# claudiok/clsim

Measured on AMD Instinct MI355X. Metric: propagated photons/sec (whole node), higher is better.
Workload: dtype f32

## Files before the change

clsim_amd/csrc/c_api.cpp:

```cpp
#include <cstring>
#include <map>
#include <memory>
#include <mutex>

#include "converter.h"
#include "lightsource.h"
#include "feeder.h"
#include "tabulator.h"
#include "step_store.h"
#include "flasher.h"
#include "mcpe.h"
#include "mcpe_merge.h"
#include "mcpe_union.h"
#include "pmt_hits.h"
#include "cable_shadow.h"
#include "event_stats.h"
#include "frame_photons.h"
#include "frame_photon_union.h"
#include "pmt_series.h"
#include "photon_hits.h"
#include "pmt_photon_hits.h"

using namespace clsimhip;

// ... 586 lines not shown
    long n = 0;
    const int rc = guarded_const(c, [&] { need(c, "converter"); need(name, "name"); n = c->impl.get_table(name, out, cap); });
    return rc == CLSIMHIP_OK ? n : rc;
}
static void copy_launched(const clsimhip::KLaunched &l, int out[6])
{
    out[0] = l.family; out[1] = l.lengths; out[2] = l.tilt; out[3] = l.aniso; out[4] = l.flasher; out[5] = l.fast;
}
int clsimhip_get_last_launch(const clsimhip_converter *c, int out[6])
{
    return guarded_const(c, [&] { need(c, "converter"); need(out, "out"); copy_launched(c->impl.last_launch(), out); });
}
int clsimhip_get_rng_state(clsimhip_converter *c, uint64_t *x_out, size_t count)
{
    return guarded(c, [&] { need(c, "converter"); c->impl.get_rng_state(x_out, count); });
}
int clsimhip_debug_counters(clsimhip_converter *c, uint32_t out[4])
{
    return guarded(c, [&] { need(c, "converter"); c->impl.debug_counters(out); });
}
int clsimhip_eval_device_function(clsimhip_converter *c, int what, int layer, int fast, const float *in4, size_t n, float *out4)
{
    return guarded(c, [&] { need(c, "converter"); c->impl.eval_device_function(what, layer, fast != 0, in4, n, out4); });
}
int clsimhip_eval_device_random(clsimhip_converter *c, int what, int generator, int fast, uint64_t *x, const uint32_t *a, size_t n_streams, size_t draws,
                                float *out)
{
    return guarded(c, [&] { need(c, "converter"); c->impl.eval_device_random(what, generator, fast != 0, x, a, n_streams, draws, out); });
}
int clsimhip_eval_math(int device_ordinal, int what, const float *x, const float *y, size_t n, float *out)
{
    return guarded(nullptr, [&] {
        need(x, "x"); need(out, "out");
        int count = 0;
        if (hipGetDeviceCount(&count) != hipSuccess || count <= 0) throw Error(CLSIMHIP_ERR_DEVICE, "no HIP device available");
        DeviceGuard on_device(device_ordinal);
        DeviceBuffer<float> bx(n + 4, "hipMalloc"), by, bout(n + 4, "hipMalloc");
        float *dx = bx.get(), *dy = nullptr, *dout = bout.get();
        hip_check(hipMemcpy(dx, x, n * 4, hipMemcpyHostToDevice), "hipMemcpy");
        if (y) {
            by.alloc(n + 4, "hipMalloc");
            dy = by.get();
            hip_check(hipMemcpy(dy, y, n * 4, hipMemcpyHostToDevice), "hipMemcpy");
        }
        hip_check(launch_eval_math(what, dx, dy, static_cast<uint32_t>(n), dout, nullptr), "eval_math launch");
        hip_check(hipDeviceSynchronize(), "eval_math");
        hip_check(hipMemcpy(out, dout, n * 4, hipMemcpyDeviceToHost), "hipMemcpy");
    });
}
int clsimhip_check_math_exhaustive(int device_ordinal, int what, int exp_lo, int exp_hi, uint32_t *result, size_t result_cap)
{
    return guarded(nullptr, [&] {
        need(result, "result");
        if (!((what >= 11 && what <= 13) || (what >= 16 && what <= 19)) || exp_lo < -126 || exp_hi > 127 || exp_lo > exp_hi || result_cap < 1 || result_cap > 4096)
            throw Error(CLSIMHIP_ERR_CONFIG, "clsimhip_check_math_exhaustive: what in 11..13 or 16..19, -126 <= exp_lo <= exp_hi <= 127, 1 <= result_cap <= 4096");
        int count = 0;
        if (hipGetDeviceCount(&count) != hipSuccess || count <= 0) throw Error(CLSIMHIP_ERR_DEVICE, "no HIP device available");
        DeviceGuard on_device(device_ordinal);
        DeviceBuffer<uint32_t> buf(result_cap, "hipMalloc");
        hip_check(hipMemset(buf.get(), 0, result_cap * 4), "hipMemset");
        hip_check(launch_check_math(what, exp_lo, exp_hi, buf.get(), static_cast<uint32_t>(result_cap), nullptr), "check_math launch");
        hip_check(hipDeviceSynchronize(), "check_math");
        hip_check(hipMemcpy(result, buf.get(), result_cap * 4, hipMemcpyDeviceToHost), "hipMemcpy");
    });
}


namespace {
void plan_steps(const clsimhip_step_request *requests, size_t n, size_t granularity, std::vector<uint64_t> &first, uint64_t &real, uint64_t &padded)
{
    need(requests, "requests");
    if (granularity == 0) throw Error(CLSIMHIP_ERR_ARGUMENT, "granularity must not be 0");
    first.assign(n + 1, 0);
    for (size_t i = 0; i < n; ++i) {
        const clsimhip_step_request &q = requests[i];
        if (q.kind > CLSIMHIP_STEPS_MUON) throw Error(CLSIMHIP_ERR_ARGUMENT, "unknown step request kind");
        if (q.photons_per_step == 0 && q.num_steps > 0) throw Error(CLSIMHIP_ERR_ARGUMENT, "photonsPerStep may not be <= 0!");
        if (q.kind == CLSIMHIP_STEPS_CASCADE && !(q.pa > 0.f)) throw Error(CLSIMHIP_ERR_ARGUMENT, "cascade shape parameter must be positive");
        first[i + 1] = first[i] + q.num_steps + (q.num_photons_in_last_step > 0 ? 1 : 0);
    }
    real = first[n];
    padded = ((real + granularity - 1) / granularity) * granularity;
}
}

extern "C" {
int clsimhip_count_generated_steps(const clsimhip_step_request *requests, size_t n, size_t granularity, size_t *steps_out, size_t *padded_out)
{
    return guarded(nullptr, [&] {
        std::vector<uint64_t> first; uint64_t real = 0, padded = 0;
        plan_steps(requests, n, granularity, first, real, padded);
        if (steps_out) *steps_out = static_cast<size_t>(real);
        if (padded_out) *padded_out = static_cast<size_t>(padded);
    });
}
int clsimhip_generate_steps_device(int device, const clsimhip_step_request *requests, size_t n, uint64_t seed, size_t granularity,
                                   void *d_steps, size_t capacity, void *hip_stream, size_t *padded_out)
{
    return guarded(nullptr, [&] {
        need(d_steps, "d_steps");
        std::vector<uint64_t> first; uint64_t real = 0, padded = 0;
        plan_steps(requests, n, granularity, first, real, padded);
        if (padded > capacity) throw Error(CLSIMHIP_ERR_ARGUMENT, "the requests produce more steps than the buffer holds");
        if (padded_out) *padded_out = static_cast<size_t>(padded);
        if (padded == 0) return;
        int count = 0;
        if (hipGetDeviceCount(&count) != hipSuccess || count <= 0) throw Error(CLSIMHIP_ERR_DEVICE, "no HIP device available (the step producer has no CPU fallback)");
        DeviceGuard on_device(device);
// ... 767 lines not shown
```

clsim_amd/csrc/detmath.hip.h:

```cpp
#pragma once
#ifndef __HIPCC_RTC__
#include <hip/hip_runtime.h>
#include <stdint.h>
#endif

#include "math_tables.h"

#define DM __device__ __forceinline__

namespace dm {

DM float fma_(float a, float b, float c) { return __builtin_fmaf(a, b, c); }
DM float sqrt_(float a) { return __builtin_sqrtf(a); }
DM float rsqrt_(float a) { return 1.0f / __builtin_sqrtf(a); }
DM float rint_(float a) { return __builtin_rintf(a); }

DM uint32_t f2u(float f) { return __builtin_bit_cast(uint32_t, f); }
DM float u2f(uint32_t u) { return __builtin_bit_cast(float, u); }

DM float rcp_(float x)
{
    const float r0 = __builtin_amdgcn_rcpf(x);
    const float e0 = fma_(-x, r0, 1.0f);
    return fma_(e0, r0, r0);
}
DM float rcp_of_rcp_(float b, float x)
{
    const float e = fma_(-b, x, 1.0f);
    return fma_(e, x, x);
}
DM bool div_near_ok_(float a) { return __builtin_fabsf(a) >= 9.094947017729282e-13f; }
DM float div_near_with_(float a, float b, float y)
{
    const float q0 = a * y;
    const float r0 = fma_(-b, q0, a);
    const float q1 = fma_(r0, y, q0);
    const float r1 = fma_(-b, q1, a);
    return fma_(r1, y, q1);
}
DM float div_near_(float a, float b) { return div_near_with_(a, b, rcp_(b)); }
DM float sqrt_near_(float x)
{
    const float s = __builtin_amdgcn_sqrtf(x);
    const uint32_t dn = __builtin_elementwise_sub_sat(f2u(s), 1u);
    const float s_dn = u2f(dn), s_up = u2f(f2u(s) + 1u);
    const float r_dn = fma_(-s_dn, s, x);
    const float r_up = fma_(-s_up, s, x);
    uint32_t m_dn, m_up;
    asm("v_med3_i32 %0, %1, 0, 1" : "=v"(m_dn) : "v"(r_dn));
    asm("v_med3_i32 %0, %1, 0, 1" : "=v"(m_up) : "v"(r_up));
    return u2f(dn + m_dn + m_up);
}
DM float rsqrt_near_(float x) { return rcp_(sqrt_near_(x)); }
DM bool rsqrt_unit_ok_(float x) { return (f2u(x) - (0x3f800000u - 1023u)) <= 2046u; }
DM float rsqrt_unit_(float x)
{
    const int d = (int)(f2u(x) - 0x3f800000u);
    const uint32_t above = 0x3f800000u - ((uint32_t)d & ~1u);
    const uint32_t below = 0x3f800000u + ((uint32_t)(3 - d) >> 2);
    return u2f((d < 0) ? below : above);
}

constexpr uint32_t kMathLogWords = 4u * MT_LOG_ROWS, kMathScWords = 2u * MT_SC_ROWS, kMathTableWords = (kMathLogWords + kMathScWords + 3u) & ~3u;
static __device__ const float kLogTable[kMathLogWords] = MT_LOG_TABLE;
static __device__ const float kScTable[kMathScWords] = MT_SC_TABLE;
static const float kLogTableHost[kMathLogWords] = MT_LOG_TABLE;
static const float kScTableHost[kMathScWords] = MT_SC_TABLE;

constexpr float LN2_HI = 0.693359375f;
constexpr float LN2_LO = -2.12194440e-4f;
constexpr float LOG2E = 1.44269504088896341f;

DM float log_poly(float r)
{
    float p = 7.0376836292e-2f;
    p = fma_(p, r, -1.1514610310e-1f);
    p = fma_(p, r, 1.1676998740e-1f);
    p = fma_(p, r, -1.2420140846e-1f);
    p = fma_(p, r, 1.4249322787e-1f);
    p = fma_(p, r, -1.6668057665e-1f);
    p = fma_(p, r, 2.0000714765e-1f);
    p = fma_(p, r, -2.4999993993e-1f);
    p = fma_(p, r, 3.3333331174e-1f);
    return p;
}

DM float frexp_sqrt2(float x, int &e)
{
    const uint32_t ix = f2u(x);
    const int32_t d = (int32_t)(ix - 0x3f3504f3u);
    e = d >> 23;
    return u2f(ix - ((uint32_t)e << 23));
}

struct LdsTable { uint32_t address; };
template <class Row> DM Row table_row_(const float *table, uint32_t byte_offset)
{
    return *reinterpret_cast<const Row *>(reinterpret_cast<const char *>(table) + byte_offset);
}
template <class Row> DM Row table_row_(LdsTable table, uint32_t byte_offset)
{
    typedef const Row __attribute__((address_space(3))) *lds_row_ptr;
    return *reinterpret_cast<lds_row_ptr>(static_cast<uintptr_t>(table.address + byte_offset));
}

template <class Table>
DM float log_with_(float x, Table table)
{
    typedef float row_t __attribute__((ext_vector_type(4)));
    const uint32_t ix = f2u(x);
    const float m = u2f((ix & 0x007fffffu) | 0x3f800000u);
    const float fe = (float)__builtin_amdgcn_frexp_expf(x);
    const row_t row = table_row_<row_t>(table, (ix >> 14) & 0x1f0u);
// ... 206 lines not shown
```

clsim_amd/csrc/prop_aux_kernels.hip:

```cpp
#include <hip/hip_runtime.h>

#include "prop_device.hip.h"
#include "prop_launch.h"

namespace clsimhip {

__global__ void __launch_bounds__(256) scan_steps_kernel(const DevStep *steps, uint32_t n, uint32_t *meta, WorkRecord *work,
                                                         const uint64_t *rng_x, const uint32_t *rng_a, uint32_t num_generators)
{
    uint32_t m = 0;
    for (uint32_t i = blockIdx.x * 256 + threadIdx.x; i < n; i += gridDim.x * 256) {
        WorkRecord r;
        r.step = steps[i];
        r.x = rng_x[i];
        r.a = rng_a[i];
        r.done = 0u;
        {
            const float f[8] = {r.step.x, r.step.y, r.step.z, r.step.t, r.step.theta, r.step.phi, r.step.length, r.step.beta};
            bool finite = true;
#pragma unroll
            for (int k = 0; k < 8; ++k) finite = finite && (__builtin_fabsf(f[k]) <= 3.0e38f);
            const bool no_spectrum = (num_generators > 1u) && ((r.step.source_type_and_pad & 0xffu) >= num_generators);
            if ((!finite || no_spectrum) && r.step.num_photons != 0u) { r.step.num_photons = 0u; atomicAdd(meta + 2, 1u); }
        }
// ... 134 lines not shown
                        const uint32_t k2 = atomicAdd(result, 1u);
                        if (k2 + 2u < result_cap && (k2 & 1u) == 0u) { result[k2 + 1u] = dm::f2u(a); result[k2 + 2u] = dm::f2u(b); }
                    }
                }
            }
        }
        return;
    }
    for (int e = exp_lo; e <= exp_hi; ++e) {
        const uint32_t bits = ((uint32_t)(e + 127) << 23) | m;
        for (int sign = 0; sign < ((what == 11 || what == 17) ? 2 : 1); ++sign) {
            const float x = dm::u2f(bits | ((uint32_t)sign << 31));
            float want, got;
            if (what == 18) {
                if (e != exp_lo || sign != 0 || m > 2046u) continue;
                const float xx = dm::u2f(0x3f800000u - 1023u + m);
                want = 1.0f / __builtin_sqrtf(xx); got = dm::rsqrt_unit_(xx);
                if (!dm::rsqrt_unit_ok_(xx) || dm::rsqrt_unit_ok_(dm::u2f(0x3f800000u + 1024u)) || dm::rsqrt_unit_ok_(dm::u2f(0x3f800000u - 1024u))) got = 0.0f;
                if (dm::f2u(want) != dm::f2u(got)) { const uint32_t k = atomicAdd(result, 1u); if (k + 1u < result_cap) result[k + 1u] = dm::f2u(xx); }
                continue;
            }
            if (what == 17) { const float b = 1.0f / x; want = 1.0f / b; got = dm::rcp_of_rcp_(dm::rcp_(x), x); }
            else if (what == 11) { want = 1.0f / x; got = dm::rcp_(x); }
            else if (what == 12) { want = __builtin_sqrtf(x); got = dm::sqrt_near_(x); }
            else { want = 1.0f / __builtin_sqrtf(x); got = dm::rsqrt_near_(x); }
            if (dm::f2u(want) != dm::f2u(got)) {
                const uint32_t k = atomicAdd(result, 1u);
                if (k + 1u < result_cap) result[k + 1u] = dm::f2u(x);
            }
        }
    }
}

hipError_t launch_scan_steps(const KParams &P, hipStream_t stream)
{
    const uint32_t sgrid = (P.n_steps + 255u) / 256u;
    hipLaunchKernelGGL(scan_steps_kernel, dim3(sgrid < 1024u ? sgrid : 1024u), dim3(256), 0, stream, P.steps, P.n_steps, P.queue,
                       P.work, P.rng_x, P.rng_a, (uint32_t)P.num_gen);
    return hipGetLastError();
}

hipError_t launch_assemble_hits(const KParams &P, bool flasher, hipStream_t stream)
{
    const size_t image_bytes = (size_t)P.table_words * 4;
    const void *kernel = flasher ? reinterpret_cast<const void *>(&assemble_hits_kernel<true>) : reinterpret_cast<const void *>(&assemble_hits_kernel<false>);
    if (const hipError_t e = allow_dynamic_lds(kernel, image_bytes)) return e;
    if (flasher) hipLaunchKernelGGL((assemble_hits_kernel<true>), dim3(512), dim3(256), image_bytes, stream, P);
    else hipLaunchKernelGGL((assemble_hits_kernel<false>), dim3(512), dim3(256), image_bytes, stream, P);
    return hipGetLastError();
}

hipError_t launch_check_math(int what, int exp_lo, int exp_hi, uint32_t *result, uint32_t result_cap, hipStream_t stream)
{
    hipLaunchKernelGGL(check_math_kernel, dim3((1u << 23) / 256), dim3(256), 0, stream, what, exp_lo, exp_hi, result, result_cap);
    return hipGetLastError();
}

hipError_t launch_eval_math(int what, const float *xs, const float *ys, uint32_t n, float *out, hipStream_t stream)
{
    if (n == 0) return hipSuccess;
    hipLaunchKernelGGL(eval_math_kernel, dim3((n + 255) / 256), dim3(256), 0, stream, what, xs, ys, n, out);
    return hipGetLastError();
}

}
```

clsim_amd/csrc/prop_device.hip.h:

```cpp
#pragma once
#ifndef __HIPCC_RTC__
#include <hip/hip_runtime.h>
#endif

#include "detmath.hip.h"
#include "../../include/clsimhip.h"
#include "kparams.h"
#include "instrument.hip.h"

namespace clsimhip {

#ifndef CLSIMHIP_BLOCK
#define CLSIMHIP_BLOCK 256
#define CLSIMHIP_MIN_WAVES 7
#endif
constexpr int kBlock = CLSIMHIP_BLOCK;
constexpr int kMinWavesPerSimd = CLSIMHIP_MIN_WAVES;
constexpr int kWavesPerBlock = kBlock / 64;
constexpr int kStageRecords = 8;
constexpr int kStubWords = 16;
#ifndef CLSIMHIP_PRIO_SHIFT
#define CLSIMHIP_PRIO_SHIFT 1
#endif
constexpr int kPrioShift = CLSIMHIP_PRIO_SHIFT;
constexpr int kTabSlots = 512;
#ifndef CLSIMHIP_TAB_POOL
#define CLSIMHIP_TAB_POOL 448
#endif
constexpr int kTabPool = CLSIMHIP_TAB_POOL;
constexpr int kTabSegWords = 12;
constexpr int kTabWaveWords = 2 * kTabPool + 2 * 64 * kTabSegWords;
static_assert(kTabWaveWords >= 2 * kTabSlots + 64 && kTabWaveWords % 4 == 0, "table maker: a wave's LDS region");
constexpr float kEpsilon = 0.00001f;
constexpr float kSpeedOfLight = 0.299792458f;
constexpr float kPi = 3.14159265359f;
constexpr uint32_t kNoStep = 0xffffffffu;
constexpr int kTiltScalarBins = 6;

typedef const __attribute__((address_space(4))) KParams *KP;

DM KP fresh_params(KP p)
{
    asm volatile("" : "+s"(p));
    return p;
}

extern __shared__ __attribute__((aligned(16))) uint32_t lds_words[];

DM uint64_t ballot(bool p) { return __builtin_amdgcn_ballot_w64(p); }

struct Rec4 { float a, b, c, d; };

enum CensusRegion { kCensusCrossing = 0, kCensusFilter = 1, kCensusLiu = 2, kCensusHG = 3, kCensusSearchFull = 4, kCensusSearchNamed = 5,
                    kCensusCreation = 6, kCensusService = 7, kCensusScatter = 8, kCensusWalk = 9, kCensusAim = 10, kCensusRegions = 16 };

DM float lds_log(float x) { return dm::log_with_(x, dm::LdsTable{0u}); }
DM void lds_sincos_2pi(float x, float &s, float &c) { dm::sincos_2pi_with_(x, s, c, dm::LdsTable{4u * dm::kMathLogWords}); }

DM float ldsf(uint32_t i) { return __builtin_bit_cast(float, lds_words[i]); }
DM uint32_t ldsu(uint32_t i) { return lds_words[i]; }
DM Rec4 lds_rec4(uint32_t i) { return *reinterpret_cast<const Rec4 *>(&lds_words[i]); }
#ifdef KPARAMS_BAKED
DM Rec4 lds_rec4_wide(uint32_t i)
{
    typedef float f32x4 __attribute__((ext_vector_type(4)));
    typedef const f32x4 __attribute__((address_space(3))) *lds_vec_ptr;
    const f32x4 v = *reinterpret_cast<lds_vec_ptr>(static_cast<uintptr_t>(4u * i));
    return Rec4{v.x, v.y, v.z, v.w};
}
DM float ldsf_at_byte(uint32_t byte)
{
    typedef const float __attribute__((address_space(3))) *lds_float_ptr;
    return *reinterpret_cast<lds_float_ptr>(static_cast<uintptr_t>(byte));
}
#endif
DM uint32_t lds_u16(uint32_t off, uint32_t i)
{
    const uint32_t w = lds_words[off + (i >> 1)];
    return (i & 1) ? (w >> 16) : (w & 0xffffu);
}

DM float rng_co(uint64_t &x, uint32_t a)
{
    x = (x & 0xffffffffull) * (uint64_t)a + (x >> 32);
    const uint32_t lo = (uint32_t)x;
    float t;
    asm volatile("s_setreg_imm32_b32 hwreg(HW_REG_MODE, 0, 2), 3\n\t"
                 "v_cvt_f32_u32_e32 %0, %1\n\t"
                 "s_setreg_imm32_b32 hwreg(HW_REG_MODE, 0, 2), 0"
                 : "=v"(t) : "v"(lo));
    return t * 2.3283064365386963e-10f;
}
DM float rng_oc(uint64_t &x, uint32_t a) { return 1.0f - rng_co(x, a); }

DM float sqr(float a) { return a * a; }
DM float div_by(float a, float b, float r, bool ok)
{
    if (ok) {
        const float q = a * r;
        return dm::fma_(dm::fma_(-b, q, a), r, q);
    }
    return a / b;
}
DM float rcp_sel(float x, bool fast) { return fast ? dm::rcp_(x) : 1.0f / x; }
constexpr uint32_t kFastLengths = 32u, kFastMatrices = 64u, kFastAniso = 128u;
template <bool FAST>
DM float div_by_t(float a, float b, float r, bool ok)
{
    if (FAST) { const float q = a * r; return dm::fma_(dm::fma_(-b, q, a), r, q); }
    return div_by(a, b, r, ok);
}
template <bool FAST>
DM float rcp_t(float x, bool fast) { return FAST ? dm::rcp_(x) : rcp_sel(x, fast); }
DM float clampf(float v, float lo, float hi) { v = (v > lo) ? v : lo; return (v < hi) ? v : hi; }
DM int clampi(int v, int lo, int hi) { v = (v > lo) ? v : lo; return (v < hi) ? v : hi; }
DM float clampf_ordered(float v, float lo, float hi) { return __builtin_amdgcn_fmed3f(v, lo, hi); }
DM int clamp_index(int v, int hi)
{
#ifdef KPARAMS_BAKED
    if (__builtin_constant_p(hi)) return clampi(v, 0, hi);
#endif
// ... 167 lines not shown
}
template <bool FAST = false>
DM float scattering_cos(KP P, uint64_t &x, uint32_t a)
{
    const ScatterK K = scatter_constants(P);
    const float rr = rng_co(x, a);
    if (!FAST) {
        const int kind = P->scatter_kind;
        if (kind == 0) return hg_cos(K, rr);
        if (kind == 1) return liu_cos(K, rr);
    }
    const uint32_t ok = FAST ? 0xffu : K.div_ok;
    CENSUS_REGION(P, kCensusScatter);
    if (rr < K.mix_frac) {
        CENSUS_REGION(P, kCensusLiu);
        return liu_cos<FAST>(K, div_by_t<FAST>(rr, K.mix_frac, K.rcp_mix_frac, (ok & 4u) != 0));
    }
    CENSUS_REGION(P, kCensusHG);
    return hg_cos<FAST>(K, div_by_t<FAST>(1.0f - rr, K.mix_frac_rest, K.rcp_mix_frac_rest, (ok & 8u) != 0));
}

template <bool FAST = false>
DM float abs_len_corr(KP P, const Vec3 &d)
{
    const float n0 = (P->an_azx * d.x) + (P->an_azy * d.y);
    const float n1 = (P->an_mazy * d.x) + (P->an_azx * d.y);
    const float s0 = n0 * n0, s1 = n1 * n1, s2 = d.z * d.z;
    const float nB = (s0 * P->an_rl[0] + s1 * P->an_rl[1]) + s2 * P->an_rl[2];
    const float An = (s0 * P->an_l[0] + s1 * P->an_l[1]) + s2 * P->an_l[2];
    const float x = (P->an_B2 - nB) * An;
    return (FAST || (P->div_ok & kFastAniso) != 0u) ? 2.0f * dm::rcp_(x) : 2.0f / x;
}
template <typename M>
DM void apply_matrix(M m, int renorm, Vec3 &d, bool fast)
{
    const float x = (m[0] * d.x) + (m[1] * d.y) + (m[2] * d.z);
    const float y = (m[3] * d.x) + (m[4] * d.y) + (m[5] * d.z);
    const float z = (m[6] * d.x) + (m[7] * d.y) + (m[8] * d.z);
    d.x = x; d.y = y; d.z = z;
    if (renorm) {
        const float n2 = d.x * d.x + d.y * d.y + d.z * d.z;
        const float norm = fast ? dm::rsqrt_near_(n2) : dm::rsqrt_(n2);
        d.x = d.x * norm; d.y = d.y * norm; d.z = d.z * norm;
    }
}

template <bool FAST = false>
DM float tilt_z_shift(KP P, float px, float py, float pz)
{
    const float z_rescaled = div_by_t<FAST>(pz - P->tilt_first_z, P->tilt_dz, P->rcp_tilt_dz, (P->div_ok & 1u) != 0);
    const int nz = P->tilt_nz, nd = P->tilt_nd;
    const uint32_t off_dist = P->off_tilt_dist;
#ifdef KPARAMS_BAKED
    const int k = clamp_index((int)z_rescaled, nz - 2);
#else
    const int k = clamp_index((int)__builtin_floorf(z_rescaled), nz - 2);
#endif
    const float fraction_z_above = z_rescaled - (float)k;
    const float fraction_z_below = 1.0f - fraction_z_above;
    const float nr = P->tilt_lnx * px + P->tilt_lny * py;
    int j = 1;
    if (FAST || nd <= kTiltScalarBins + 2) {
#ifdef KPARAMS_BAKED
#pragma unroll
        for (int t = 0; t < kTiltScalarBins; ++t)
            if (t < nd - 2) j += (nr >= P->tilt_inner_dist[t]) ? 1 : 0;
#else
#pragma unroll
        for (int t = 0; t < kTiltScalarBins; ++t) j += (nr >= P->tilt_inner_dist[t]) ? 1 : 0;
#endif
    } else {
        for (int t = 1; t < nd - 1; ++t) j += (nr >= ldsf(off_dist + t)) ? 1 : 0;
    }
#ifdef KPARAMS_BAKED
    const Rec4 bin = (KParams::off_tilt_bins % 4u == 0u) ? lds_rec4_wide(P->off_tilt_bins + 4u * (uint32_t)j) : lds_rec4(P->off_tilt_bins + 4u * (uint32_t)j);
#else
    const Rec4 bin = lds_rec4(P->off_tilt_bins + 4u * (uint32_t)j);
#endif
    const float thisDist = bin.a;
    const float q = (thisDist - nr) * bin.c;
    float frac_at_lower = dm::fma_(dm::fma_(-bin.b, q, thisDist - nr), bin.c, q);
    if (!FAST && __builtin_bit_cast(uint32_t, bin.d) == 0u) frac_at_lower = (thisDist - nr) / bin.b;
    const float frac_at_upper = 1.0f - frac_at_lower;
#ifdef KPARAMS_BAKED
    if (FAST) {
        const uint32_t at = (__builtin_bit_cast(uint32_t, bin.d) >> 1) + 4u * (uint32_t)k;
        const uint32_t up = 4u * (uint32_t)nz;
        const float val_at_lower = (ldsf_at_byte(at + 4u) * fraction_z_above + ldsf_at_byte(at) * fraction_z_below);
        const float val_at_upper = (ldsf_at_byte(at + up + 4u) * fraction_z_above + ldsf_at_byte(at + up) * fraction_z_below);
        return (val_at_upper * frac_at_upper + val_at_lower * frac_at_lower);
    }
#endif
    const uint32_t lo = P->off_tilt_zcorr + (uint32_t)((j - 1) * nz + k);
    const uint32_t hi = lo + (uint32_t)nz;
    const float val_at_lower = (ldsf(lo + 1) * fraction_z_above + ldsf(lo) * fraction_z_below);
    const float val_at_upper = (ldsf(hi + 1) * fraction_z_above + ldsf(hi) * fraction_z_below);
    return (val_at_upper * frac_at_upper + val_at_lower * frac_at_lower);
}

DM float generate_wavelength(KP P, int gen, uint64_t &x, uint32_t a)
{
    if (P->gen_kind[gen] == 1) return P->gen_value[gen];
    if (P->gen_kind[gen] == 2) {
        const float u = rng_oc(x, a);
        return 1.0f / (P->gen_first[gen] + u * P->gen_spacing[gen]);
    }
    const float r = rng_oc(x, a);
// ... 136 lines not shown
    Birth b;
    const float shift = st.length * rng_co(rx, ra);
    const float inv_speed = 1.0f / (kSpeedOfLight * st.beta);
    b.x = st.x + step_dir.x * shift;
    b.y = st.y + step_dir.y * shift;
    b.z = st.z + step_dir.z * shift;
    b.t = st.t + inv_speed * shift;
    const uint32_t source_type = st.source_type_and_pad & 0xffu;
    b.d = step_dir;
    if (!FLASHER || source_type == 0) {
        const float wavelength = generate_wavelength(P, 0, rx, ra);
        const float rcp = 1.0f / (st.beta * phase_ref_index(P, wavelength));
        const float cos_c = (rcp < 1.0f) ? rcp : 1.0f;
        const float sin_c = dm::sqrt_near_(1.0f - cos_c * cos_c);
        b.wlen = wavelength;
        scatter_direction(cos_c, sin_c, b.d, rng_co(rx, ra));
    } else {
        b.wlen = (source_type < (uint32_t)P->num_gen) ? generate_wavelength(P, (int)source_type, rx, ra) : 0.0f;
    }
    b.abs_lens_initial = P->has_fixed_abs ? P->fixed_abs : -lds_log(rng_oc(rx, ra));
    return b;
}

template <int MED, bool TILT, bool FLASHER, bool TAB, bool FAST = false>
DM void create_photon(KP P, const DevStep *step_ptr, const Vec3 &step_dir, uint64_t &rx, uint32_t ra, Photon &ph)
{
    CENSUS_REGION(P, kCensusCreation);
    ph.rx_start = rx;
    const Birth b = photon_birth<FLASHER>(P, step_ptr, step_dir, rx, ra);
    if (TAB) { ph.tab_remainder = P->tab_volume_step * rng_oc(rx, ra); ph.tab_depth = 0.0f; ph.tab_wlen = b.wlen; }
    ph.px = b.x; ph.py = b.y; ph.pz = b.z; ph.pt = b.t;
    ph.d = b.d;
    ph.num_scatters = 0;
    ph.total_path = 0.0f;
    if (!TILT) ph.layer = clamp_index((int)div_by_t<FAST>(ph.pz - P->layer_bottom, P->layer_thickness, P->rcp_layer_thickness, (P->div_ok & 2u) != 0), P->num_layers - 1);
    ph.inv_groupvel = 1.0f / group_velocity<FAST>(P, b.wlen);
    ph.abs_lens_left = b.abs_lens_initial;
    ph.ice = ice_factors<MED>(P, b.wlen);
}

template <int MED, bool TILT, bool ANISO, bool FAST = false>
DM float propagate_through_layers(KP P, Photon &ph, uint64_t &rx, uint32_t ra)
{
    const float thickness = P->layer_thickness, bottom = P->layer_bottom;
    const int num_layers = P->num_layers;
    const uint32_t off_layers = P->off_layers;
    const float *len_table = (MED == CLSIMHIP_LENGTHS_TABLE) ? P->len_table : nullptr;
    const bool fast = FAST || (P->div_ok & kFastLengths) != 0u;
    CENSUS_REGION(P, kCensusWalk);
    float effective_z;
    int current_layer;
    if (TILT) {
        effective_z = ph.pz - tilt_z_shift<FAST>(P, ph.px, ph.py, ph.pz);
        current_layer = clamp_index((int)div_by_t<FAST>(effective_z - bottom, thickness, P->rcp_layer_thickness, (P->div_ok & 2u) != 0), num_layers - 1);
    } else {
        effective_z = ph.pz - P->tilt_const;
        current_layer = ph.layer;
    }
    const float dz = ph.d.z;
    const float corr = (ANISO && P->has_abs_corr) ? abs_len_corr<FAST>(P, ph.d) : 1.0f;
    if (ANISO) ph.abs_lens_left *= corr;
    const float lower = ((float)current_layer * thickness) + bottom;
    float boundary = (dz < 0.0f) ? lower : (lower + thickness);
    const float sca_step_left = -lds_log(rng_oc(rx, ra));
    float sca_len, abs_len, rcp_sca = 0.0f, rcp_abs = 0.0f;
    const bool seeded = (MED == CLSIMHIP_LENGTHS_ICECUBE) && fast;
#ifdef KPARAMS_BAKED
    if (MED != CLSIMHIP_LENGTHS_TABLE) {
        const uint32_t at = off_layers + 4u * (uint32_t)current_layer;
        const Rec4 r = (KParams::off_layers % 4u == 0u) ? lds_rec4_wide(at) : lds_rec4(at);
        layer_lengths_of<MED, FAST>(r, ph.ice, sca_len, abs_len, rcp_sca, rcp_abs, fast);
        boundary = (dz < 0.0f) ? r.d : (r.d + thickness);
    } else
#endif
    layer_lengths<MED, FAST>(off_layers, len_table, ph.ice, current_layer, sca_len, abs_len, rcp_sca, rcp_abs, fast);
    const float recip_thickness = P->recip_thickness;
    const float to_boundary = boundary - effective_z;
    float over_sca, over_abs;
    if (__builtin_expect(fast && (ballot(!dm::div_near_ok_(to_boundary)) == 0ull), 1)) {
        over_sca = seeded ? dm::div_near_with_(to_boundary, sca_len, rcp_sca) : dm::div_near_(to_boundary, sca_len);
        over_abs = seeded ? dm::div_near_with_(to_boundary, abs_len, rcp_abs) : dm::div_near_(to_boundary, abs_len);
    } else {
        over_sca = to_boundary / sca_len;
        over_abs = to_boundary / abs_len;
    }
    float ais = (dz * sca_step_left - over_sca) * recip_thickness;
    float aia = (dz * ph.abs_lens_left - over_abs) * recip_thickness;
    int j = current_layer;
    {
        const bool down = (dz < 0.0f);
        const float sgn = down ? -1.0f : 1.0f;
        const int step = down ? -1 : 1;
        const int last = down ? 0 : (num_layers - 1);
        const float signed_thickness = sgn * thickness;
        while ((j != last) && (sgn * ais > 0.0f) && (sgn * aia > 0.0f)) {
            CENSUS_REGION(P, kCensusCrossing);
            j += step;
            boundary += signed_thickness;
            layer_lengths<MED, FAST>(off_layers, len_table, ph.ice, j, sca_len, abs_len, rcp_sca, rcp_abs, fast);
            ais -= sgn * (seeded ? rcp_sca : rcp_t<FAST>(sca_len, fast));
            aia -= sgn * (seeded ? rcp_abs : rcp_t<FAST>(abs_len, fast));
        }
    }
    float distance, to_absorption;
    if ((current_layer == j) || (__builtin_fabsf(dz) < kEpsilon)) {
        distance = sca_step_left * sca_len;
        to_absorption = ph.abs_lens_left * abs_len;
    } else {
        const float recip_dz = dm::rcp_(dz);
        distance = (ais * thickness * sca_len + boundary - effective_z) * recip_dz;
        to_absorption = (aia * thickness * abs_len + boundary - effective_z) * recip_dz;
    }
    if (!TILT) ph.layer = j;
    if (to_absorption < distance) {
        distance = to_absorption;
        ph.abs_lens_left = 0.0f;
    } else {
        const float left = to_absorption - distance;
        ph.abs_lens_left = __builtin_expect(fast && (ballot(!dm::div_near_ok_(left)) == 0ull), 1) ? (seeded ? dm::div_near_with_(left, abs_len, rcp_abs) : dm::div_near_(left, abs_len)) : left / abs_len;
    }
    if (ANISO) ph.abs_lens_left = ph.abs_lens_left / corr;
    return distance;
}

struct Detector {
    uint32_t off_strings, off_sets, off_layer_to_om;
    int max_layers;
    float string_max_radius_sq, string_max_radius, om_radius_sq, pancake;
    int has_pancake;
};

DM void collide_with_string(KP P, const Detector &D, uint32_t s, float dir_len_xy_sqr, const Photon &ph, float &step_len,
                            bool &hit, uint32_t &hit_string, uint32_t &hit_dom)
{
    const Rec4 str = lds_rec4(D.off_strings + 8u * s);
    const float wx = str.a - ph.px, wy = str.b - ph.py;
    {
        const float smin = sqr((ph.px - str.a) * ph.d.y - (ph.py - str.b) * ph.d.x) / dir_len_xy_sqr;
        if (smin > D.string_max_radius_sq) return;
    }
    {
        const float along = wx * ph.d.x + wy * ph.d.y;
        const float ex = wx - step_len * ph.d.x, ey = wy - step_len * ph.d.y;
        const float reach = D.string_max_radius + (1e-3f + 9.5367431640625e-7f * (__builtin_fabsf(ph.px) + __builtin_fabsf(ph.py) + __builtin_fabsf(str.a) + __builtin_fabsf(str.b)));
        const float reach_sq = reach * reach;
        if ((along <= 0.0f) && (wx * wx + wy * wy > reach_sq)) return;
        if ((along >= step_len * dir_len_xy_sqr) && (ex * ex + ey * ey > reach_sq)) return;
    }
    if ((ph.d.z > 0.0f) && (ph.pz > str.c)) return;
    if ((ph.d.z < 0.0f) && (ph.pz < str.d)) return;
    const uint32_t set = ldsu(D.off_strings + 8u * s + 4) & 0xffu;
    const Rec4 lay = lds_rec4(D.off_sets + 4u * set);
    const float start_z = lay.b, height = lay.c;
    const int nl = (int)__builtin_bit_cast(uint32_t, lay.a);
    int low = (int)((ph.pz - start_z) / height);
    int high = (int)((ph.pz + ph.d.z * step_len - start_z) / height);
    if (high < low) { const int tmp = low; low = high; high = tmp; }
    low = clampi(low, 0, nl - 1);
    high = clampi(high, 0, nl - 1);
    const uint32_t base = set * (uint32_t)D.max_layers;
    for (int layer = low; layer <= high; ++layer) {
        const uint32_t dom = lds_u16(D.off_layer_to_om, base + (uint32_t)layer);
        if (dom == 0xFFFFu) continue;
        float dom_x, dom_y, dom_z;
        dom_position(P, s, dom, dom_x, dom_y, dom_z);
        const float dx = dom_x - ph.px, dy = dom_y - ph.py, dzz = dom_z - ph.pz;
        const float dr2 = (dx * dx + dy * dy) + dzz * dzz;
        const float urdot = (dx * ph.d.x + dy * ph.d.y) + dzz * ph.d.z;
        float discr = sqr(urdot) - dr2 + D.om_radius_sq;
        if (discr < 0.0f) continue;
        discr = D.has_pancake ? (dm::sqrt_(discr) / D.pancake) : dm::sqrt_(discr);
        if (urdot + discr < 0.0f) continue;
        const float smin1 = urdot - discr;
        if (smin1 < 0.0f) continue;
        if (smin1 < step_len) {
            step_len = smin1;
            hit_string = s;
            hit_dom = dom;
            hit = true;
        }
    }
}

DM uint32_t free_flight_bound(KP P, float x, float y)
{
    const int n = P->prox_n;
    const int ix = clamp_index((int)((x - P->prox_x0) * P->prox_inv_cell), n - 1);
    const int iy = clamp_index((int)((y - P->prox_y0) * P->prox_inv_cell), n - 1);
    return P->prox_map[(uint32_t)iy * (uint32_t)n + (uint32_t)ix];
}
DM float free_flight_of(uint32_t word) { return (float)(word & 0xffu) * 0.25f; }

DM bool segment_misses_string(KP P, const Photon &ph, float len, uint32_t word)
{
    CENSUS_REGION(P, kCensusAim);
    const uint32_t s = word >> 16;
    if (s == 0xffffu) return false;
    if (!(len < (float)((word >> 8) & 0xffu) * 0.25f)) return false;
    const Rec4 str = lds_rec4(P->off_strings + 8u * s);
    const float wx = str.a - ph.px, wy = str.b - ph.py;
    const float reach = P->prox_reach + (1e-3f + 9.5367431640625e-7f * (__builtin_fabsf(ph.px) + __builtin_fabsf(ph.py) + __builtin_fabsf(str.a) + __builtin_fabsf(str.b)));
    const float reach_sq = reach * reach;
    const float along = wx * ph.d.x + wy * ph.d.y;
    const float cross = wx * ph.d.y - wy * ph.d.x;
    const float m = ph.d.x * ph.d.x + ph.d.y * ph.d.y;
    const bool behind = (along <= 0.0f) && (wx * wx + wy * wy > reach_sq);
    const bool beside = cross * cross > (m * reach_sq) * 1.0001f;
    return behind || beside;
}

constexpr uint32_t kSearchNone = 0u, kSearchFull = 1u, kSearchNamed = 2u;
template <bool INSIDE = false>
DM uint32_t dom_search_needed(KP P, const Photon &ph, float len)
{
    CENSUS_REGION(P, kCensusFilter);
    const float inv = P->dprox_inv_cell;
    const int ny = P->dprox_ny, nz = P->dprox_nz;
    const int ix = clamp_index((int)((ph.px - P->dprox_x0) * inv), P->dprox_nx - 1);
    const int iy = clamp_index((int)((ph.py - P->dprox_y0) * inv), ny - 1);
    const int iz = clamp_index((int)((ph.pz - P->dprox_z0) * inv), nz - 1);
    const uint4 cell = P->dom_cells[((uint32_t)ix * (uint32_t)ny + (uint32_t)iy) * (uint32_t)nz + (uint32_t)iz];
    const uint32_t w = cell.x;
    const float others = (float)((w >> 16) & 0xffu) * 0.25f;
    if (!(len < others)) return kSearchFull;
    const uint32_t id = w & 0xffffu;
    if (id == 0xffffu) return kSearchNone;
    const float wx = dm::u2f(cell.y) - ph.px, wy = dm::u2f(cell.z) - ph.py, wz = dm::u2f(cell.w) - ph.pz;
    const float urdot = (wx * ph.d.x + wy * ph.d.y) + wz * ph.d.z;
    if (urdot < 0.0f) return kSearchNone;
    if (INSIDE) {
        const float room = P->om_radius_sq - ((wx * wx + wy * wy) + wz * wz);
        const float p = P->has_pancake ? P->pancake : 1.0f;
        if ((p * p - 1.0f) * (urdot * urdot) < room * 0.999f - 1e-5f) return kSearchNone;
    }
    const float along = clampf_ordered(urdot, 0.0f, len);
    const float qx = wx - along * ph.d.x, qy = wy - along * ph.d.y, qz = wz - along * ph.d.z;
    const float reach = P->dprox_radius + 0.01f;
    return ((qx * qx + qy * qy) + qz * qz > reach * reach) ? kSearchNone : (kSearchNamed + id);
}

template <bool FAST = false>
DM bool find_collision_named(KP P, const Photon &ph, float &step_len, uint32_t id, const uint4 named, uint32_t &hit_string, uint32_t &hit_dom)
{
    CENSUS_REGION(P, kCensusSearchNamed);
    const float dir_len_xy_sqr = sqr(ph.d.x) + sqr(ph.d.y);
    if (dir_len_xy_sqr <= 0.0f) return false;
    const uint32_t s = named.x & 0xffffu, dom = named.x >> 16;
    const int cell_x0 = (int)(named.y & 0xfffu), cell_y0 = (int)((named.y >> 12) & 0xfffu);
    const int cell_x1 = (int)(named.w & 0xfffu), cell_y1 = (int)((named.w >> 12) & 0xfffu);
    const uint32_t sd = named.y >> 24;
    {
        const uint32_t off_subdet = P->off_subdet;
        const Rec4 g0 = lds_rec4(off_subdet + 12u * sd);
        const Rec4 g1 = lds_rec4(off_subdet + 12u * sd + 4u);
        const Rec4 g2 = lds_rec4(off_subdet + 12u * sd + 8u);
        const int nx = (int)__builtin_bit_cast(uint32_t, g0.a), ny = (int)__builtin_bit_cast(uint32_t, g0.b);
        const float wx = g0.c, wy = g0.d, sx = g1.a, sy = g1.b;
        const uint32_t proven = FAST ? 3u : __builtin_bit_cast(uint32_t, g1.d);
        const bool okx = (proven & 1u) != 0, oky = (proven & 2u) != 0;
        int low_x, low_y, high_x, high_y;
        if (FAST) {
            low_x = (int)div_by_t<true>(ph.px - sx, wx, g2.a, true);
            low_y = (int)div_by_t<true>(ph.py - sy, wy, g2.b, true);
            high_x = (int)div_by_t<true>(ph.px + ph.d.x * step_len - sx, wx, g2.a, true);
            high_y = (int)div_by_t<true>(ph.py + ph.d.y * step_len - sy, wy, g2.b, true);
        } else {
            const float ax = ph.px - sx, ay = ph.py - sy, bx = ph.px + ph.d.x * step_len - sx, by = ph.py + ph.d.y * step_len - sy;
            low_x = (int)(okx ? div_by_t<true>(ax, wx, g2.a, true) : ax / wx);
            low_y = (int)(oky ? div_by_t<true>(ay, wy, g2.b, true) : ay / wy);
            high_x = (int)(okx ? div_by_t<true>(bx, wx, g2.a, true) : bx / wx);
            high_y = (int)(oky ? div_by_t<true>(by, wy, g2.b, true) : by / wy);
        }
        if (high_x < low_x) { const int tmp = low_x; low_x = high_x; high_x = tmp; }
// ... 269 lines not shown
```

clsim_amd/csrc/prop_launch.h:

```cpp
#pragma once
#include <hip/hip_runtime_api.h>
#include <hip/hip_vector_types.h>

#include <map>
#include <mutex>
#include <tuple>
#include <type_traits>

#include "../../include/clsimhip.h"
#include "kparams.h"

namespace clsimhip {

hipError_t launch_prop_kernel(const KParams &P, const KVariant &v, hipStream_t stream);
size_t prop_kernel_lds_bytes(uint32_t table_words);
int prop_kernel_block_size();
size_t prop_kernel_max_lanes();
size_t prop_kernel_lds_budget();
hipError_t launch_keep_kernel(const KParams &P, const KVariant &v, hipStream_t stream);
hipError_t launch_tab_kernel(const KParams &P, const KVariant &v, hipStream_t stream);
hipError_t launch_pool_kernel(const KParams &P, const KVariant &v, hipStream_t stream);
bool pool_kernel_fits(uint32_t table_words, uint32_t keep_strings, int num_layers);
size_t pool_kernel_max_steps();
hipError_t launch_pool_keep_kernel(const KParams &P, const KVariant &v, hipStream_t stream);
hipError_t launch_scan_steps(const KParams &P, hipStream_t stream);
hipError_t launch_assemble_hits(const KParams &P, bool flasher, hipStream_t stream);
hipError_t launch_eval_math(int what, const float *xs, const float *ys, uint32_t n, float *out, hipStream_t stream);
hipError_t launch_check_math(int what, int exp_lo, int exp_hi, uint32_t *result, uint32_t result_cap, hipStream_t stream);
hipError_t launch_eval_function(const KParams &P, int lengths_kind, bool has_tilt, bool fast, int what, int layer, const float4 *in, uint32_t n, float4 *out,
                                hipStream_t stream);
hipError_t launch_eval_random(const KParams &P, bool fast, int what, int generator, uint64_t *x, const uint32_t *a, uint32_t n_streams, uint32_t draws,
                              float *out, hipStream_t stream);
hipError_t launch_generate_flasher_steps(const clsimhip_flasher_config &cfg, const clsimhip_flasher_request *d_requests, const void *d_plan,
                                         uint32_t n_requests, uint64_t total, uint64_t seed, const float *d_profiles, void *d_out,
                                         hipStream_t stream);
hipError_t launch_generate_steps(const clsimhip_step_request *d_requests, const uint64_t *d_first_step, uint32_t n_requests,
                                 uint64_t total_real, uint64_t total_padded, uint64_t seed, void *d_out, hipStream_t stream);

inline hipError_t check_lengths(const KParams &P, const KVariant &v)
{
    if (v.lengths < CLSIMHIP_LENGTHS_CONSTANT || v.lengths > CLSIMHIP_LENGTHS_TABLE) return hipErrorInvalidValue;
    if (v.lengths == CLSIMHIP_LENGTHS_TABLE && (!P.len_table || P.len_tab_n < 2)) return hipErrorInvalidValue;
    return hipSuccess;
}

template <typename F>
hipError_t dispatch_lengths(int lengths, F &&f)
{
    switch (lengths) {
    case CLSIMHIP_LENGTHS_CONSTANT: return f(std::integral_constant<int, CLSIMHIP_LENGTHS_CONSTANT>{});
    case CLSIMHIP_LENGTHS_ICECUBE: return f(std::integral_constant<int, CLSIMHIP_LENGTHS_ICECUBE>{});
    case CLSIMHIP_LENGTHS_TABLE: return f(std::integral_constant<int, CLSIMHIP_LENGTHS_TABLE>{});
    }
    return hipErrorInvalidValue;
}
template <typename F> hipError_t dispatch_switch(bool on, F &&f) { return !on ? f(std::false_type{}) : f(std::true_type{}); }
template <typename F> hipError_t dispatch_fast(bool fast, F &&f) { return fast ? f(std::true_type{}) : f(std::false_type{}); }
template <bool ALWAYS_FLASHER = false, typename F>
hipError_t dispatch_variant(const KVariant &v, bool fast, F &&f)
{
    return dispatch_lengths(v.lengths, [&](auto lengths) {
        return dispatch_switch(v.tilt, [&](auto tilt) {
            return dispatch_switch(v.aniso, [&](auto aniso) {
                const auto rest = [&](auto flasher) {
                    return dispatch_fast(fast, [&](auto fast_tag) { return f(lengths, tilt, aniso, flasher, fast_tag); });
                };
                if constexpr (ALWAYS_FLASHER) return rest(std::true_type{});
                else return dispatch_switch(v.flasher, rest);
            });
        });
    });
}

struct LaunchPlan { int cus = 0, resident = 0; };
inline hipError_t plan_launch(const void *kernel, int block, size_t lds_bytes, LaunchPlan &plan)
{
    static std::mutex mutex;
    static std::map<std::tuple<int, const void *, int, size_t>, LaunchPlan> plans;
    int device = 0;
    if (const hipError_t e = hipGetDevice(&device)) return e;
    std::lock_guard<std::mutex> lk(mutex);
// ... 23 lines not shown
```

Baseline: 4.350 billion.

## Use cvt+min index clamps and byte-offset layer walk in baked kernels

In baked-parameter builds, float-to-index clamps for tilt, layer, proximity and DOM grid lookups become an unsigned convert followed by a min against a compile-time bound, emitted as inline asm. The layer-crossing loop is rewritten to step a byte offset into the LDS layer records, folding the direction sign into the remaining-length accumulators so each iteration does fewer compares and less address arithmetic. An exhaustive checker kernel (what=20) is added to confirm the asm clamp matches the reference clamp. The goal is fewer ALU instructions on the hot propagation path. The tradeoff is that negative-input saturation now depends on the exact semantics of the hardware convert instruction.

```diff
diff --git a/clsim_amd/csrc/c_api.cpp b/clsim_amd/csrc/c_api.cpp
--- a/clsim_amd/csrc/c_api.cpp
+++ b/clsim_amd/csrc/c_api.cpp
@@ -662,8 +662,8 @@
 {
     return guarded(nullptr, [&] {
         need(result, "result");
-        if (!((what >= 11 && what <= 13) || (what >= 16 && what <= 19)) || exp_lo < -126 || exp_hi > 127 || exp_lo > exp_hi || result_cap < 1 || result_cap > 4096)
-            throw Error(CLSIMHIP_ERR_CONFIG, "clsimhip_check_math_exhaustive: what in 11..13 or 16..19, -126 <= exp_lo <= exp_hi <= 127, 1 <= result_cap <= 4096");
+        if (!((what >= 11 && what <= 13) || (what >= 16 && what <= 20)) || exp_lo < -126 || exp_hi > 127 || exp_lo > exp_hi || result_cap < 1 || result_cap > 4096)
+            throw Error(CLSIMHIP_ERR_CONFIG, "clsimhip_check_math_exhaustive: what in 11..13 or 16..20, -126 <= exp_lo <= exp_hi <= 127, 1 <= result_cap <= 4096");
         int count = 0;
         if (hipGetDeviceCount(&count) != hipSuccess || count <= 0) throw Error(CLSIMHIP_ERR_DEVICE, "no HIP device available");
         DeviceGuard on_device(device_ordinal);
diff --git a/clsim_amd/csrc/detmath.hip.h b/clsim_amd/csrc/detmath.hip.h
--- a/clsim_amd/csrc/detmath.hip.h
+++ b/clsim_amd/csrc/detmath.hip.h
@@ -59,6 +59,15 @@
     const uint32_t above = 0x3f800000u - ((uint32_t)d & ~1u);
     const uint32_t below = 0x3f800000u + ((uint32_t)(3 - d) >> 2);
     return u2f((d < 0) ? below : above);
+}
+template <int HI>
+DM int clamp_index_of(float f)
+{
+    if (HI < 0) { const int v = (int)f, lo = (v > 0) ? v : 0; return (lo < HI) ? lo : HI; }
+    uint32_t r;
+    asm("v_cvt_u32_f32_e32 %0, %1\n\t"
+        "v_min_u32_e32 %0, %2, %0" : "=v"(r) : "v"(f), "n"((uint32_t)HI));
+    return (int)r;
 }
 
 constexpr uint32_t kMathLogWords = 4u * MT_LOG_ROWS, kMathScWords = 2u * MT_SC_ROWS, kMathTableWords = (kMathLogWords + kMathScWords + 3u) & ~3u;
diff --git a/clsim_amd/csrc/index_clamp_check_kernel.hip b/clsim_amd/csrc/index_clamp_check_kernel.hip
--- /dev/null
+++ b/clsim_amd/csrc/index_clamp_check_kernel.hip
@@ -0,0 +1,39 @@
+#include <hip/hip_runtime.h>
+
+#include "detmath.hip.h"
+#include "prop_launch.h"
+
+namespace clsimhip {
+
+template <int HI>
+DM void check_index_clamp_one(float f, uint32_t *result, uint32_t result_cap)
+{
+    const int hi = __builtin_amdgcn_readfirstlane(HI);
+    const int v = (int)f, lo = (v > 0) ? v : 0, want = (lo < hi) ? lo : hi;
+    if (dm::clamp_index_of<HI>(f) != want) {
+        const uint32_t k = atomicAdd(result, 1u);
+        if (k + 1u < result_cap) result[k + 1u] = dm::f2u(f);
+    }
+}
+__global__ void check_index_clamp_kernel(uint32_t *result, uint32_t result_cap)
+{
+    const uint32_t m = blockIdx.x * blockDim.x + threadIdx.x;
+    if (m >= (1u << 23)) return;
+    for (uint32_t k = 0; k < 512u; ++k) {
+        const float f = dm::u2f((m << 9) | k);
+        check_index_clamp_one<0>(f, result, result_cap);
+        check_index_clamp_one<1>(f, result, result_cap);
+        check_index_clamp_one<0xa8>(f, result, result_cap);
+        check_index_clamp_one<0xaa>(f, result, result_cap);
+        check_index_clamp_one<0x1ff>(f, result, result_cap);
+        check_index_clamp_one<0x3fff>(f, result, result_cap);
+    }
+}
+
+hipError_t launch_check_index_clamp(uint32_t *result, uint32_t result_cap, hipStream_t stream)
+{
+    hipLaunchKernelGGL(check_index_clamp_kernel, dim3((1u << 23) / 256), dim3(256), 0, stream, result, result_cap);
+    return hipGetLastError();
+}
+
+}
diff --git a/clsim_amd/csrc/prop_aux_kernels.hip b/clsim_amd/csrc/prop_aux_kernels.hip
--- a/clsim_amd/csrc/prop_aux_kernels.hip
+++ b/clsim_amd/csrc/prop_aux_kernels.hip
@@ -210,6 +210,7 @@
 
 hipError_t launch_check_math(int what, int exp_lo, int exp_hi, uint32_t *result, uint32_t result_cap, hipStream_t stream)
 {
+    if (what == 20) return launch_check_index_clamp(result, result_cap, stream);
     hipLaunchKernelGGL(check_math_kernel, dim3((1u << 23) / 256), dim3(256), 0, stream, what, exp_lo, exp_hi, result, result_cap);
     return hipGetLastError();
 }
diff --git a/clsim_amd/csrc/prop_device.hip.h b/clsim_amd/csrc/prop_device.hip.h
--- a/clsim_amd/csrc/prop_device.hip.h
+++ b/clsim_amd/csrc/prop_device.hip.h
@@ -67,6 +67,18 @@
     typedef const f32x4 __attribute__((address_space(3))) *lds_vec_ptr;
     const f32x4 v = *reinterpret_cast<lds_vec_ptr>(static_cast<uintptr_t>(4u * i));
     return Rec4{v.x, v.y, v.z, v.w};
+}
+DM Rec4 lds_rec4_wide_at_byte(uint32_t byte)
+{
+    typedef float f32x4 __attribute__((ext_vector_type(4)));
+    typedef const f32x4 __attribute__((address_space(3))) *lds_vec_ptr;
+    const f32x4 v = *reinterpret_cast<lds_vec_ptr>(static_cast<uintptr_t>(byte));
+    return Rec4{v.x, v.y, v.z, v.w};
+}
+DM Rec4 lds_rec4_at_byte(uint32_t byte)
+{
+    typedef const Rec4 __attribute__((address_space(3))) *lds_rec_ptr;
+    return *reinterpret_cast<lds_rec_ptr>(static_cast<uintptr_t>(byte));
 }
 DM float ldsf_at_byte(uint32_t byte)
 {
@@ -340,7 +352,7 @@
     const int nz = P->tilt_nz, nd = P->tilt_nd;
     const uint32_t off_dist = P->off_tilt_dist;
 #ifdef KPARAMS_BAKED
-    const int k = clamp_index((int)z_rescaled, nz - 2);
+    const int k = dm::clamp_index_of<KParams::tilt_nz - 2>(z_rescaled);
 #else
     const int k = clamp_index((int)__builtin_floorf(z_rescaled), nz - 2);
 #endif
@@ -583,7 +595,11 @@
     int current_layer;
     if (TILT) {
         effective_z = ph.pz - tilt_z_shift<FAST>(P, ph.px, ph.py, ph.pz);
+#ifdef KPARAMS_BAKED
+        current_layer = dm::clamp_index_of<KParams::num_layers - 1>(div_by_t<FAST>(effective_z - bottom, thickness, P->rcp_layer_thickness, (P->div_ok & 2u) != 0));
+#else
         current_layer = clamp_index((int)div_by_t<FAST>(effective_z - bottom, thickness, P->rcp_layer_thickness, (P->div_ok & 2u) != 0), num_layers - 1);
+#endif
     } else {
         effective_z = ph.pz - P->tilt_const;
         current_layer = ph.layer;
@@ -617,6 +633,42 @@
     }
     float ais = (dz * sca_step_left - over_sca) * recip_thickness;
     float aia = (dz * ph.abs_lens_left - over_abs) * recip_thickness;
+#ifdef KPARAMS_BAKED
+    const bool down = (dz < 0.0f);
+    const float sgn = down ? -1.0f : 1.0f;
+    const float signed_thickness = sgn * thickness;
+    float S_s = sgn * ais, S_a = sgn * aia;
+    constexpr bool kRecordsInLds = (MED != CLSIMHIP_LENGTHS_TABLE);
+    constexpr uint32_t kAtUnit = kRecordsInLds ? 16u : 1u;
+    const uint32_t at_start = kAtUnit * (uint32_t)current_layer;
+    const uint32_t at_step = down ? (0u - kAtUnit) : kAtUnit;
+    const uint32_t at_last = down ? 0u : kAtUnit * (uint32_t)(num_layers - 1);
+    uint32_t at = at_start;
+    const bool crossing = (at != at_last) && (S_s > 0.0f) && (S_a > 0.0f);
+    if (crossing) do {
+        CENSUS_REGION(P, kCensusCrossing);
+        at += at_step;
+        boundary += signed_thickness;
+        if (kRecordsInLds) {
+            const Rec4 r = (KParams::off_layers % 4u == 0u) ? lds_rec4_wide_at_byte(4u * off_layers + at) : lds_rec4_at_byte(4u * off_layers + at);
+            layer_lengths_of<MED, FAST>(r, ph.ice, sca_len, abs_len, rcp_sca, rcp_abs, fast);
+        } else {
+            layer_lengths<MED, FAST>(off_layers, len_table, ph.ice, (int)at, sca_len, abs_len, rcp_sca, rcp_abs, fast);
+        }
+        S_s -= seeded ? rcp_sca : rcp_t<FAST>(sca_len, fast);
+        S_a -= seeded ? rcp_abs : rcp_t<FAST>(abs_len, fast);
+    } while ((at != at_last) && (S_s > 0.0f) && (S_a > 0.0f));
+    float distance, to_absorption;
+    if (!crossing || (__builtin_fabsf(dz) < kEpsilon)) {
+        distance = sca_step_left * sca_len;
+        to_absorption = ph.abs_lens_left * abs_len;
+    } else {
+        const float recip_dz = dm::rcp_(dz);
+        distance = (S_s * signed_thickness * sca_len + boundary - effective_z) * recip_dz;
+        to_absorption = (S_a * signed_thickness * abs_len + boundary - effective_z) * recip_dz;
+    }
+    if (!TILT) ph.layer = (int)(at / kAtUnit);
+#else
     int j = current_layer;
     {
         const bool down = (dz < 0.0f);
@@ -643,6 +695,7 @@
         to_absorption = (aia * thickness * abs_len + boundary - effective_z) * recip_dz;
     }
     if (!TILT) ph.layer = j;
+#endif
     if (to_absorption < distance) {
         distance = to_absorption;
         ph.abs_lens_left = 0.0f;
@@ -716,8 +769,13 @@
 DM uint32_t free_flight_bound(KP P, float x, float y)
 {
     const int n = P->prox_n;
+#ifdef KPARAMS_BAKED
+    const int ix = dm::clamp_index_of<KParams::prox_n - 1>((x - P->prox_x0) * P->prox_inv_cell);
+    const int iy = dm::clamp_index_of<KParams::prox_n - 1>((y - P->prox_y0) * P->prox_inv_cell);
+#else
     const int ix = clamp_index((int)((x - P->prox_x0) * P->prox_inv_cell), n - 1);
     const int iy = clamp_index((int)((y - P->prox_y0) * P->prox_inv_cell), n - 1);
+#endif
     return P->prox_map[(uint32_t)iy * (uint32_t)n + (uint32_t)ix];
 }
 DM float free_flight_of(uint32_t word) { return (float)(word & 0xffu) * 0.25f; }
@@ -747,9 +805,15 @@
     CENSUS_REGION(P, kCensusFilter);
     const float inv = P->dprox_inv_cell;
     const int ny = P->dprox_ny, nz = P->dprox_nz;
+#ifdef KPARAMS_BAKED
+    const int ix = dm::clamp_index_of<KParams::dprox_nx - 1>((ph.px - P->dprox_x0) * inv);
+    const int iy = dm::clamp_index_of<KParams::dprox_ny - 1>((ph.py - P->dprox_y0) * inv);
+    const int iz = dm::clamp_index_of<KParams::dprox_nz - 1>((ph.pz - P->dprox_z0) * inv);
+#else
     const int ix = clamp_index((int)((ph.px - P->dprox_x0) * inv), P->dprox_nx - 1);
     const int iy = clamp_index((int)((ph.py - P->dprox_y0) * inv), ny - 1);
     const int iz = clamp_index((int)((ph.pz - P->dprox_z0) * inv), nz - 1);
+#endif
     const uint4 cell = P->dom_cells[((uint32_t)ix * (uint32_t)ny + (uint32_t)iy) * (uint32_t)nz + (uint32_t)iz];
     const uint32_t w = cell.x;
     const float others = (float)((w >> 16) & 0xffu) * 0.25f;
diff --git a/clsim_amd/csrc/prop_launch.h b/clsim_amd/csrc/prop_launch.h
--- a/clsim_amd/csrc/prop_launch.h
+++ b/clsim_amd/csrc/prop_launch.h
@@ -27,6 +27,7 @@
 hipError_t launch_assemble_hits(const KParams &P, bool flasher, hipStream_t stream);
 hipError_t launch_eval_math(int what, const float *xs, const float *ys, uint32_t n, float *out, hipStream_t stream);
 hipError_t launch_check_math(int what, int exp_lo, int exp_hi, uint32_t *result, uint32_t result_cap, hipStream_t stream);
+hipError_t launch_check_index_clamp(uint32_t *result, uint32_t result_cap, hipStream_t stream);
 hipError_t launch_eval_function(const KParams &P, int lengths_kind, bool has_tilt, bool fast, int what, int layer, const float4 *in, uint32_t n, float4 *out,
                                 hipStream_t stream);
 hipError_t launch_eval_random(const KParams &P, bool fast, int what, int generator, uint64_t *x, const uint32_t *a, uint32_t n_streams, uint32_t draws,
```

Result: faster. 4.416 billion (median of 6 runs) (+1.5%).
